# indiejoseph/speech-distill

Measured on AMD Instinct MI355X. Metric: distill-step tokens/sec (student seq_len=512), higher is better.
Workload: dtype bf16; 1 GPU; BASELINE config 2: Qwen3-0.6B-shape student + SoulX-1.7B-shape teacher (random init), V=159488, batch 4/GPU, seq_len 512, top_k 128, T=2.0 alpha=0.5, student fwd+bwd + teacher fwd + top-K + KL/CE; global_batch=4, seq_len=512, parallelism=single

## Files before the change

### speech_distill_amd/csrc/sd_attn.hip

```cpp
#include <type_traits>
#include "sd_common.cuh"
#include "../../include/sd_hip.h"
#include "sd_prof.h"
#include "sd_debug.h"
#include "sd_events.h"

namespace {

constexpr int D = 128;
constexpr int TILE = 64 * D * 2;
constexpr float NEG = -1.0e30f;
constexpr float LOG2E = 1.4426950408889634f;

SD_DEV int f_swz(int row) { return ((row & 3) << 2) | ((row >> 2) & 3); }

template <int NP = 4>
struct TileDma {
  int voff[NP];
  long row_bytes;
#if defined(__HIP_DEVICE_COMPILE__)
  __amdgpu_buffer_rsrc_t rsrc;
#endif
  SD_DEV void init(const bf16* g, long ld, int rows, int w, int lane) {
    row_bytes = ld * 2;
#if defined(__HIP_DEVICE_COMPILE__)
    rsrc = __builtin_amdgcn_make_buffer_rsrc((void*)g, 0, (int)(((long)(rows - 1) * ld + D) * 2), 0x00020000);
#endif
#pragma unroll
    for (int i = 0; i < NP; ++i) {
      const int p = (w * NP + i) * 64 + lane;
      const int row = p >> 4, s = p & 15;
      voff[i] = (int)(((long)row * ld + ((s ^ f_swz(row)) * 8)) * 2);
    }
  }
  SD_DEV void issue(int row0, char* lds, int w) const {
#if defined(__HIP_DEVICE_COMPILE__)
    const int soff = (int)(row0 * row_bytes);
#pragma unroll
    for (int i = 0; i < NP; ++i)
      __builtin_amdgcn_raw_ptr_buffer_load_lds(rsrc, (SD_LDS void*)(lds + (w * NP + i) * 1024), 16, voff[i], soff, 0, 0);
#endif
  }
};

SD_DEV bf16x8 row_frag(const char* lds, int row0, int st, int lane) {
  const int row = row0 + (lane & 31);
  const int ch = 2 * st + (lane >> 5);
  return *(const bf16x8*)(lds + row * 256 + ((ch ^ f_swz(row)) << 4));
}

SD_DEV void tr_frag4(const char* lds, int rb, int lane, bf16x8 (&out)[4]) {
  const int gi = lane >> 4, i = lane & 15, q4 = i >> 2, pp = i & 3;
  const int rA = rb + 4 * (gi >> 1) + q4, rB = rA + 8;
  const int sA = f_swz(rA), sB = f_swz(rB);
  const unsigned base = lds_addr(lds) + 8 * (pp & 1);
  const unsigned aA = base + rA * 256, aB = base + rB * 256;
  const int chl = (gi & 1) * 2 + (pp >> 1);
  sd_u64 raw[8];
#pragma unroll
  for (int db = 0; db < 4; ++db) {
    const int ch = db * 4 + chl;
    lds_tr16_pair_asm(raw[2 * db], raw[2 * db + 1], aA + ((ch ^ sA) << 4), aB + ((ch ^ sB) << 4));
  }
  lds_tr_wait8(raw);
#pragma unroll
  for (int db = 0; db < 4; ++db) out[db] = cat8_u64(raw[2 * db], raw[2 * db + 1]);
}

SD_DEV void tr_issue4(const char* lds, int rb, int lane, sd_u64 (&raw)[8]) {
  const int gi = lane >> 4, i = lane & 15, q4 = i >> 2, pp = i & 3;
  const int rA = rb + 4 * (gi >> 1) + q4, rB = rA + 8;
  const int sA = f_swz(rA), sB = f_swz(rB);
  const unsigned base = lds_addr(lds) + 8 * (pp & 1);
  const unsigned aA = base + rA * 256, aB = base + rB * 256;
  const int chl = (gi & 1) * 2 + (pp >> 1);
#pragma unroll
  for (int db = 0; db < 4; ++db) {
    const int ch = db * 4 + chl;
    lds_tr16_pair_asm(raw[2 * db], raw[2 * db + 1], aA + ((ch ^ sA) << 4), aB + ((ch ^ sB) << 4));
  }
}
SD_DEV void tr_finish4(sd_u64 (&raw)[8], bf16x8 (&out)[4]) {
  lds_tr_wait8(raw);
#pragma unroll
  for (int db = 0; db < 4; ++db) out[db] = cat8_u64(raw[2 * db], raw[2 * db + 1]);
}

SD_DEV float halves_max(float x) {
  float a = x, b = x;
  asm volatile("s_nop 1\n\tv_permlane32_swap_b32 %0, %1\n\ts_nop 0" : "+v"(a), "+v"(b));
  return fmaxf(a, b);
}

SD_DEV bf16x8 acc_frag(const f32x16& p, int s) {
  bf16x8 r;
#pragma unroll
  for (int j = 0; j < 8; ++j) r[j] = (bf16)p[8 * s + j];
  return r;
}

SD_DEV int acc_row(int reg, int h) { return (reg & 3) + 8 * (reg >> 2) + 4 * h; }

SD_DEV void store_tile_rows(char* img, const f32x16 (&acc)[4], float mul, bf16* g_row0, long ld, int rows_valid, int lane) {
  const int r = lane & 31, h = lane >> 5;
  const int swr = f_swz(r);
#pragma unroll
  for (int db = 0; db < 4; ++db)
#pragma unroll
    for (int g4 = 0; g4 < 4; ++g4) {
      bf16x4 v;
#pragma unroll
      for (int e = 0; e < 4; ++e) v[e] = (bf16)(acc[db][4 * g4 + e] * mul);
      *(bf16x4*)(img + r * 256 + (((db * 4 + g4) ^ swr) << 4) + 8 * h) = v;
    }
  asm volatile("s_waitcnt lgkmcnt(0)" ::: "memory");
  const int ch = lane & 15;
#pragma unroll
  for (int i = 0; i < 8; ++i) {
    const int row = 4 * i + (lane >> 4);
    const bf16x8 v = *(const bf16x8*)(img + row * 256 + ((ch ^ f_swz(row)) << 4));
    if (row < rows_valid) *(bf16x8*)(g_row0 + (long)row * ld + ch * 8) = v;
  }
}

struct AttnWg { int pair, member_head, hkv, b; };
SD_DEV AttnWg attn_wg(int id, int npairs, int heads_per_group, int Hkv, int B) {
  const int gs = npairs * heads_per_group, ng = Hkv * B;
  int g, mem;
  if ((ng & 7) == 0) {
    const int xcd = id & 7, slot = id >> 3;
    g = xcd + 8 * (slot / gs);
    mem = slot % gs;
  } else {
    g = id / gs;
    mem = id % gs;
  }
  AttnWg o;
  o.b = g / Hkv;
  o.hkv = g % Hkv;
  o.member_head = mem / npairs;
  o.pair = mem % npairs;
  return o;
}

#ifdef SD_STAMPS
#define SD_ATT_STAMP_PARAM , unsigned long long* stamps
#define ATT_STAMP()                                                                                   \
  do {                                                                                                \
    if (stamping && lane == 0 && sidx < 256) stamps[w8 * 256 + sidx] = __builtin_amdgcn_s_memtime();   \
    ++sidx;                                                                                           \
  } while (0)
#define ATT_STAMP_AT(COND, SLOT)                                                                            \
  do {                                                                                                      \
    if (stamping && (COND) && lane == 0) stamps[w8 * 256 + (SLOT)] = __builtin_amdgcn_s_memtime();           \
  } while (0)
#else
#define SD_ATT_STAMP_PARAM
#define ATT_STAMP() do { } while (0)
#define ATT_STAMP_AT(COND, SLOT) do { } while (0)
#endif

__global__ __launch_bounds__(512) void attn_fwd_kernel(const bf16* __restrict__ Q, const bf16* __restrict__ Kp,
                                                       const bf16* __restrict__ Vp, bf16* __restrict__ O,
                                                       float* __restrict__ LSE, const int* __restrict__ kv_len, long ldq,
                                                       long ldk, long ldv, long ldo, int T, int Hq, int Hkv,
                                                       float scale SD_ATT_STAMP_PARAM) {
  __shared__ __attribute__((aligned(16))) char smem[8 * TILE];
  const int lane = lane_id(), w8 = wave_id_uniform();
  const int n64 = (T + 63) / 64;
  const AttnWg wg = attn_wg((int)blockIdx.x, (n64 + 1) / 2, Hq / Hkv, Hkv, (int)gridDim.x / (((n64 + 1) / 2) * Hq));
#ifdef SD_STAMPS
  const bool stamping = stamps && wg.pair == 0 && wg.member_head == 0 && wg.hkv == 0 && wg.b == 0;
  int sidx = 0;
#endif
  ATT_STAMP();
  const int grp = w8 >> 2, rb = w8 & 1, half = (w8 >> 1) & 1;
  const int w = grp * 2 + rb;
  const int tA = n64 - 1 - wg.pair, tB = wg.pair;
  const bool active = grp == 0 || tB != tA;
  const int hkv = wg.hkv, b = wg.b;
  const int hq = hkv * (Hq / Hkv) + wg.member_head;
  const int q0w = (grp == 0 ? tA : tB) * 64 + 32 * rb;
  const int r = lane & 31, h = lane >> 5;
  const long tok0 = (long)b * T;
  const bf16* qb = Q + tok0 * ldq + hq * D;
  const bf16* kb = Kp + tok0 * ldk + hkv * D;
  const bf16* vb = Vp + tok0 * ldv + hkv * D;

  const int kv_hi = min(tA * 64 + 64, T);
  const int nkv = (kv_hi + 63) / 64;
  TileDma<2> kd, vd;
  kd.init(kb, ldk, T, w8, lane);
  vd.init(vb, ldv, T, w8, lane);
  kd.issue(0, smem, w8);
  vd.issue(0, smem + TILE, w8);
  const int q = q0w + r;
  const int qc = q < T ? q : T - 1;
  bf16x8 qf[8];
#pragma unroll
  for (int st = 0; st < 8; ++st) qf[st] = *(const bf16x8*)(qb + (long)qc * ldq + 16 * st + 8 * h);
  ATT_STAMP();
  const int klen = kv_len ? max(1, min(kv_len[b], T)) : T;
  const int lim = min(q, klen - 1);

  f32x16 o[4];
#pragma unroll
  for (int db = 0; db < 4; ++db)
#pragma unroll
    for (int e = 0; e < 16; ++e) o[db][e] = 0.f;
  float m = NEG, l = 0.f;
  const float c = scale * LOG2E;

  auto visible = [&](int i) { const int kv0 = i * 64 + 32 * half; return active && kv0 < kv_hi && kv0 <= q0w + 31; };
  unsigned kfo[8], vfo[2][8];
#pragma unroll
  for (int st = 0; st < 8; ++st) {
    const int row = 32 * half + (lane & 31), ch = 2 * st + (lane >> 5);
    kfo[st] = (unsigned)(row * 256 + ((ch ^ f_swz(row)) << 4));
  }
  {
    const int gi = lane >> 4, i16 = lane & 15, q4 = i16 >> 2, pp = i16 & 3;
    const int chl = (gi & 1) * 2 + (pp >> 1);
#pragma unroll
    for (int ss = 0; ss < 2; ++ss) {
      const int rA = 32 * half + 16 * ss + 4 * (gi >> 1) + q4, rB = rA + 8;
#pragma unroll
      for (int db = 0; db < 4; ++db) {
        const int ch = db * 4 + chl;
        vfo[ss][2 * db] = (unsigned)(8 * (pp & 1) + rA * 256 + ((ch ^ f_swz(rA)) << 4));
        vfo[ss][2 * db + 1] = (unsigned)(8 * (pp & 1) + rB * 256 + ((ch ^ f_swz(rB)) << 4));
      }
    }
  }
  const unsigned smem_a = lds_addr(smem);
  auto tile = [&](int i, int stage) {
    const char* ks = smem + stage * 2 * TILE;
    const unsigned vsa = smem_a + stage * 2 * TILE + TILE;
    f32x16 s1;
#pragma unroll
    for (int e = 0; e < 16; ++e) s1[e] = 0.f;
#pragma unroll
    for (int st = 0; st < 8; ++st) s1 = mfma32(*(const bf16x8*)(ks + kfo[st]), qf[st], s1);
    ATT_STAMP_AT(i == 3, 201);
    sd_u64 rv0[8], rv1[8];
#pragma unroll
    for (int db = 0; db < 4; ++db) lds_tr16_pair_asm(rv0[2 * db], rv0[2 * db + 1], vsa + vfo[0][2 * db], vsa + vfo[0][2 * db + 1]);
#pragma unroll
    for (int db = 0; db < 4; ++db) lds_tr16_pair_asm(rv1[2 * db], rv1[2 * db + 1], vsa + vfo[1][2 * db], vsa + vfo[1][2 * db + 1]);
    const int kv0 = i * 64 + 32 * half;
    const bool need_mask = __builtin_amdgcn_readfirstlane((int)((kv0 + 31 > q0w) || (kv0 + 31 >= klen))) != 0;
    if (need_mask) {
#pragma unroll
      for (int e = 0; e < 16; ++e) s1[e] = (kv0 + acc_row(e, h)) > lim ? NEG : s1[e];
    }
    float mx = fmaxf(fmaxf(s1[0], s1[1]), s1[2]);
#pragma unroll
    for (int e = 3; e < 15; e += 2) mx = fmaxf(fmaxf(mx, s1[e]), s1[e + 1]);
    mx = fmaxf(mx, s1[15]);
    ATT_STAMP_AT(i == 3, 202);
    mx = fmaxf(mx, __shfl_xor(mx, 32, 64));
    ATT_STAMP_AT(i == 3, 203);
    const float mn = fmaxf(m, mx);
    const float alpha = __builtin_amdgcn_exp2f((m - mn) * c);
    m = mn;
    const float mnc = -mn * c;
    float rs = 0.f;
#pragma unroll
    for (int e = 0; e < 16; ++e) {
      const float p = __builtin_amdgcn_exp2f(__builtin_fmaf(s1[e], c, mnc));
      s1[e] = p;
      rs += p;
    }
    l = l * alpha + rs;
    ATT_STAMP_AT(i == 3, 204);
    if (__any(alpha != 1.f)) {
#pragma unroll
      for (int db = 0; db < 4; ++db)
#pragma unroll
        for (int e = 0; e < 16; ++e) o[db][e] *= alpha;
    }
    ATT_STAMP_AT(i == 3, 205);
    bf16x8 vt[4];
    tr_finish4(rv0, vt);
    ATT_STAMP_AT(i == 3, 206);
    const bf16x8 p0 = acc_frag(s1, 0), p1 = acc_frag(s1, 1);
#pragma unroll
    for (int db = 0; db < 4; ++db) o[db] = mfma32(vt[db], p0, o[db]);
#pragma unroll
    for (int db = 0; db < 4; ++db) o[db] = mfma32(cat8_u64(rv1[2 * db], rv1[2 * db + 1]), p1, o[db]);
    ATT_STAMP_AT(i == 3, 207);
  };
  for (int i = 0; i < nkv; ++i) {
    if (i == 0) asm volatile("s_waitcnt vmcnt(0)" ::: "memory");
    else if (i + 2 < nkv) asm volatile("s_waitcnt vmcnt(8)" ::: "memory");
    else if (i + 1 < nkv) asm volatile("s_waitcnt vmcnt(4)" ::: "memory");
    else asm volatile("s_waitcnt vmcnt(0)" ::: "memory");
    ATT_STAMP();
    __builtin_amdgcn_s_barrier();
    asm volatile("" ::: "memory");
    ATT_STAMP();
    for (int t = (i == 0 ? 1 : i + 3); t <= i + 3; ++t)
      if (t < nkv) {
        char* nx = smem + (t & 3) * 2 * TILE;
        kd.issue(t * 64, nx, w8);
        vd.issue(t * 64, nx + TILE, w8);
      }
    ATT_STAMP();
    if (visible(i)) {
      ATT_STAMP_AT(i == 3, 200);
      tile(i, i & 3);
    }
    ATT_STAMP();
  }
  asm volatile("s_waitcnt vmcnt(0)" ::: "memory");
  __syncthreads();
  ATT_STAMP();
  float* xo = (float*)smem + (long)w * 66 * 64;
  if (half == 1) {
#pragma unroll
    for (int db = 0; db < 4; ++db)
#pragma unroll
      for (int e = 0; e < 16; ++e) xo[(db * 16 + e) * 64 + lane] = o[db][e];
    xo[64 * 64 + lane] = m;
    xo[65 * 64 + lane] = l;
  }
  __syncthreads();
  if (half == 1) return;
  {
    const float m1 = xo[64 * 64 + lane], l1 = xo[65 * 64 + lane];
    const float mn = fmaxf(m, m1);
    const float a0 = __builtin_amdgcn_exp2f((m - mn) * c), a1 = __builtin_amdgcn_exp2f((m1 - mn) * c);
#pragma unroll
    for (int db = 0; db < 4; ++db)
#pragma unroll
      for (int e = 0; e < 16; ++e) o[db][e] = o[db][e] * a0 + xo[(db * 16 + e) * 64 + lane] * a1;
    l = l * a0 + l1 * a1;
    m = mn;
  }
  l += __shfl_xor(l, 32, 64);
  const float inv = 1.f / l;
  ATT_STAMP();
  if (!active) return;
  store_tile_rows((char*)xo, o, inv, O + (tok0 + q0w) * ldo + hq * D, ldo, T - q0w, lane);
  if (q < T && h == 0) LSE[((long)b * Hq + hq) * T + q] = m * scale + __logf(l);
  ATT_STAMP();
}

__global__ __launch_bounds__(512) void attn_fwd_pipe_kernel(const bf16* __restrict__ Q, const bf16* __restrict__ Kp,
                                                            const bf16* __restrict__ Vp, bf16* __restrict__ O,
                                                            float* __restrict__ LSE, const int* __restrict__ kv_len,
                                                            long ldq, long ldk, long ldv, long ldo, int T, int Hq, int Hkv,
                                                            float scale SD_ATT_STAMP_PARAM) {
  __shared__ __attribute__((aligned(16))) char smem[8 * TILE];
  const int lane = lane_id(), w8 = wave_id_uniform();
  const int n64 = (T + 63) / 64;
  const AttnWg wg = attn_wg((int)blockIdx.x, (n64 + 1) / 2, Hq / Hkv, Hkv, (int)gridDim.x / (((n64 + 1) / 2) * Hq));
#ifdef SD_STAMPS
  const bool stamping = stamps && wg.pair == 0 && wg.member_head == 0 && wg.hkv == 0 && wg.b == 0;
  int sidx = 0;
#endif
  ATT_STAMP();
  const int grp = w8 >> 2, rb = w8 & 1, half = (w8 >> 1) & 1;
  const int w = grp * 2 + rb;
  const int tA = n64 - 1 - wg.pair, tB = wg.pair;
  const bool active = grp == 0 || tB != tA;
  const int hkv = wg.hkv, b = wg.b;
  const int hq = hkv * (Hq / Hkv) + wg.member_head;
  const int q0w = (grp == 0 ? tA : tB) * 64 + 32 * rb;
  const int r = lane & 31, h = lane >> 5;
  const long tok0 = (long)b * T;
  const bf16* qb = Q + tok0 * ldq + hq * D;
  const bf16* kb = Kp + tok0 * ldk + hkv * D;
  const bf16* vb = Vp + tok0 * ldv + hkv * D;
  const int kv_hi = min(tA * 64 + 64, T);
  const int nkv = (kv_hi + 63) / 64;
  TileDma<2> kd, vd;
  kd.init(kb, ldk, T, w8, lane);
  vd.init(vb, ldv, T, w8, lane);
  kd.issue(0, smem, w8);
  vd.issue(0, smem + TILE, w8);
  const int q = q0w + r;
  const int qc = q < T ? q : T - 1;
  bf16x8 qf[8];
#pragma unroll
  for (int st = 0; st < 8; ++st) qf[st] = *(const bf16x8*)(qb + (long)qc * ldq + 16 * st + 8 * h);
  const int klen = kv_len ? max(1, min(kv_len[b], T)) : T;
  const int lim = min(q, klen - 1);

  f32x16 o[4];
#pragma unroll
  for (int db = 0; db < 4; ++db)
#pragma unroll
    for (int e = 0; e < 16; ++e) o[db][e] = 0.f;
  float m = NEG, l = 0.f;
  const float c = scale * LOG2E;
  int nvis = 0;
  if (active) {
    const int last = (q0w + 31 - 32 * half) >> 6;
    nvis = (q0w + 31 - 32 * half) < 0 ? 0 : min(last + 1, (kv_hi - 32 * half + 63) >> 6);
  }
  unsigned kf0, vf0[2][2];
  {
    const int row = 32 * half + (lane & 31);
    kf0 = (unsigned)(row * 256 + (((lane >> 5) ^ f_swz(row)) << 4));
    const int gi = lane >> 4, i16 = lane & 15, q4 = i16 >> 2, pp = i16 & 3;
    const int chl = (gi & 1) * 2 + (pp >> 1);
#pragma unroll
    for (int ss = 0; ss < 2; ++ss) {
      const int rA = 32 * half + 16 * ss + 4 * (gi >> 1) + q4, rB = rA + 8;
      vf0[ss][0] = (unsigned)(8 * (pp & 1) + rA * 256 + ((chl ^ f_swz(rA)) << 4));
      vf0[ss][1] = (unsigned)(8 * (pp & 1) + rB * 256 + ((chl ^ f_swz(rB)) << 4));
    }
  }
  const unsigned smem_a = lds_addr(smem);
  auto s_tile = [&](int stage, f32x16& s) __attribute__((always_inline)) {
    const char* ks = smem + stage * 2 * TILE;
#pragma unroll
    for (int e = 0; e < 16; ++e) s[e] = 0.f;
#pragma unroll
    for (int st = 0; st < 8; ++st) s = mfma32(*(const bf16x8*)(ks + (kf0 ^ (unsigned)(st << 5))), qf[st], s);
  };
  auto mask_max = [&](int t, f32x16& s) __attribute__((always_inline)) -> float {
    const int kv0 = t * 64 + 32 * half;
    const bool need_mask = __builtin_amdgcn_readfirstlane((int)((kv0 + 31 > q0w) || (kv0 + 31 >= klen))) != 0;
    if (need_mask) {
#pragma unroll
      for (int e = 0; e < 16; ++e) s[e] = (kv0 + acc_row(e, h)) > lim ? NEG : s[e];
    }
    float mx = fmaxf(fmaxf(s[0], s[1]), s[2]);
#pragma unroll
    for (int e = 3; e < 15; e += 2) mx = fmaxf(fmaxf(mx, s[e]), s[e + 1]);
    mx = fmaxf(mx, s[15]);
    return halves_max(mx);
  };

  asm volatile("s_waitcnt vmcnt(0)" ::: "memory");
#pragma unroll
  for (int st = 0; st < 8; ++st) {
    u32x4 t4 = __builtin_bit_cast(u32x4, qf[st]);
    asm volatile("" : "+v"(t4));
    qf[st] = __builtin_bit_cast(bf16x8, t4);
  }
  __builtin_amdgcn_s_barrier();
  asm volatile("" ::: "memory");
  for (int t = 1; t <= 2; ++t)
    if (t < nkv) {
      char* nx = smem + (t & 3) * 2 * TILE;
      kd.issue(t * 64, nx, w8);
      vd.issue(t * 64, nx + TILE, w8);
    }
  f32x16 sc, sn;
  float mx = NEG;
  if (nvis > 0) {
    s_tile(0, sc);
    mx = mask_max(0, sc);
  }
  ATT_STAMP();
  for (int i = 0; i < nkv; ++i) {
    if (i + 2 < nkv) asm volatile("s_waitcnt vmcnt(4)" ::: "memory");
    else asm volatile("s_waitcnt vmcnt(0)" ::: "memory");
    ATT_STAMP();
    __builtin_amdgcn_s_barrier();
    asm volatile("" ::: "memory");
    ATT_STAMP();
    const bool comp = i < nvis;
    const unsigned ksa = smem_a + ((i + 1) & 3) * 2 * TILE + kf0;
    const unsigned vsa = smem_a + (i & 3) * 2 * TILE + TILE;
    const unsigned va[2][2] = {{vsa + vf0[0][0], vsa + vf0[0][1]}, {vsa + vf0[1][0], vsa + vf0[1][1]}};
    u32x4 kf[8];
    sd_u64 rv0[8], rv1[8];
    if (comp) {
#pragma unroll
      for (int st = 0; st < 8; ++st) asm volatile("ds_read_b128 %0, %1" : "=&v"(kf[st]) : "v"(ksa ^ (unsigned)(st << 5)));
#pragma unroll
      for (int db = 0; db < 4; ++db) lds_tr16_pair_asm(rv0[2 * db], rv0[2 * db + 1], va[0][0] ^ (unsigned)(db << 6), va[0][1] ^ (unsigned)(db << 6));
    }
    if (i + 3 < nkv) {
      char* nx = smem + ((i + 3) & 3) * 2 * TILE;
      kd.issue((i + 3) * 64, nx, w8);
      vd.issue((i + 3) * 64, nx + TILE, w8);
    }
    ATT_STAMP();
    if (!comp) {
      ATT_STAMP();
      continue;
    }
    const float mn = fmaxf(m, mx);
    const float alpha = __builtin_amdgcn_exp2f((m - mn) * c);
    m = mn;
    const float mnc = -mn * c;
    if (__any(alpha != 1.f)) {
#pragma unroll
      for (int db = 0; db < 4; ++db)
#pragma unroll
        for (int e = 0; e < 16; ++e) o[db][e] *= alpha;
    }
    asm volatile("s_waitcnt lgkmcnt(8)"
                 : "+v"(kf[0]), "+v"(kf[1]), "+v"(kf[2]), "+v"(kf[3]), "+v"(kf[4]), "+v"(kf[5]), "+v"(kf[6]), "+v"(kf[7]));
#pragma unroll
    for (int db = 0; db < 4; ++db) lds_tr16_pair_asm(rv1[2 * db], rv1[2 * db + 1], va[1][0] ^ (unsigned)(db << 6), va[1][1] ^ (unsigned)(db << 6));
#pragma unroll
    for (int e = 0; e < 16; ++e) sn[e] = 0.f;
    float rs = 0.f;
#pragma unroll
    for (int st = 0; st < 8; ++st) {
      sn = mfma32(__builtin_bit_cast(bf16x8, kf[st]), qf[st], sn);
#pragma unroll
      for (int e = 2 * st; e < 2 * st + 2; ++e) {
        const float p = __builtin_amdgcn_exp2f(__builtin_fmaf(sc[e], c, mnc));
        sc[e] = p;
        rs += p;
      }
      __builtin_amdgcn_sched_barrier(0);
    }
    l = l * alpha + rs;
    const bf16x8 p0 = acc_frag(sc, 0), p1 = acc_frag(sc, 1);
    asm volatile("s_waitcnt lgkmcnt(8)"
                 : "+v"(rv0[0]), "+v"(rv0[1]), "+v"(rv0[2]), "+v"(rv0[3]), "+v"(rv0[4]), "+v"(rv0[5]), "+v"(rv0[6]), "+v"(rv0[7]));
#pragma unroll
    for (int db = 0; db < 4; ++db) o[db] = mfma32(cat8_u64(rv0[2 * db], rv0[2 * db + 1]), p0, o[db]);
    lds_tr_wait8(rv1);
#pragma unroll
    for (int db = 0; db < 4; ++db) o[db] = mfma32(cat8_u64(rv1[2 * db], rv1[2 * db + 1]), p1, o[db]);
    mx = mask_max(i + 1, sn);
    sc = sn;
    ATT_STAMP();
  }
  asm volatile("s_waitcnt vmcnt(0)" ::: "memory");
  __syncthreads();
  ATT_STAMP();
  float* xo = (float*)smem + (long)w * 66 * 64;
  if (half == 1) {
#pragma unroll
    for (int db = 0; db < 4; ++db)
#pragma unroll
      for (int e = 0; e < 16; ++e) xo[(db * 16 + e) * 64 + lane] = o[db][e];
    xo[64 * 64 + lane] = m;
    xo[65 * 64 + lane] = l;
  }
  __syncthreads();
  if (half == 1) return;
  {
    const float m1 = xo[64 * 64 + lane], l1 = xo[65 * 64 + lane];
    const float mn = fmaxf(m, m1);
    const float a0 = __builtin_amdgcn_exp2f((m - mn) * c), a1 = __builtin_amdgcn_exp2f((m1 - mn) * c);
#pragma unroll
    for (int db = 0; db < 4; ++db)
#pragma unroll
      for (int e = 0; e < 16; ++e) o[db][e] = o[db][e] * a0 + xo[(db * 16 + e) * 64 + lane] * a1;
    l = l * a0 + l1 * a1;
    m = mn;
  }
  l += __shfl_xor(l, 32, 64);
  const float inv = 1.f / l;
  ATT_STAMP();
  if (!active) return;
  store_tile_rows((char*)xo, o, inv, O + (tok0 + q0w) * ldo + hq * D, ldo, T - q0w, lane);
  if (q < T && h == 0) LSE[((long)b * Hq + hq) * T + q] = m * scale + __logf(l);
  ATT_STAMP();
}

__global__ __launch_bounds__(256) void attn_delta_kernel(const bf16* __restrict__ dO, const bf16* __restrict__ O,
                                                         float* __restrict__ delta, long ldo, int T, int Hq, long total) {
  const int lane = lane_id();
  const long idx = ((long)blockIdx.x * 4 + (threadIdx.x >> 6)) * 4 + (lane >> 4);
  const int j = lane & 15;
  const bool ok = idx < total;
  const long id = ok ? idx : total - 1;
  const long tok = id / Hq;
  const int hh = (int)(id % Hq);
  bf16x8 a = *(const bf16x8*)(dO + tok * ldo + hh * D + j * 8);
  bf16x8 bb = *(const bf16x8*)(O + tok * ldo + hh * D + j * 8);
  float s = 0.f;
#pragma unroll
  for (int e = 0; e < 8; ++e) s += (float)a[e] * (float)bb[e];
  s += __shfl_xor(s, 1, 64); s += __shfl_xor(s, 2, 64); s += __shfl_xor(s, 4, 64); s += __shfl_xor(s, 8, 64);
  if (ok && j == 0) {
    const long bidx = tok / T;
    const int t = (int)(tok % T);
    delta[(bidx * Hq + hh) * T + t] = s;
  }
}

__global__ __launch_bounds__(512) void attn_bwd_dq_kernel(const bf16* __restrict__ Q, const bf16* __restrict__ Kp,
                                                          const bf16* __restrict__ Vp, const bf16* __restrict__ dO,
                                                          const float* __restrict__ LSE, const float* __restrict__ delta,
                                                          bf16* __restrict__ dQ, const int* __restrict__ kv_len, long ldq,
                                                          long ldk, long ldv, long ldo, long lddq, int T, int Hq, int Hkv,
                                                          float scale) {
  __shared__ __attribute__((aligned(16))) char smem[8 * TILE];
  const int lane = lane_id(), w8 = wave_id_uniform();
  const int grp = w8 >> 2, rb = w8 & 1, half = (w8 >> 1) & 1;
  const int w = grp * 2 + rb;
  const int n64 = (T + 63) / 64;
  const AttnWg wg = attn_wg((int)blockIdx.x, (n64 + 1) / 2, Hq / Hkv, Hkv, (int)gridDim.x / (((n64 + 1) / 2) * Hq));
  const int tA = n64 - 1 - wg.pair, tB = wg.pair;
  const bool active = grp == 0 || tB != tA;
  const int hkv = wg.hkv, b = wg.b;
  const int hq = hkv * (Hq / Hkv) + wg.member_head;
  const int q0w = (grp == 0 ? tA : tB) * 64 + 32 * rb;
  const int r = lane & 31, h = lane >> 5;
  const int klen = kv_len ? max(1, min(kv_len[b], T)) : T;
  const long tok0 = (long)b * T;
  const bf16* qb = Q + tok0 * ldq + hq * D;
  const bf16* kb = Kp + tok0 * ldk + hkv * D;
  const bf16* vb = Vp + tok0 * ldv + hkv * D;
  const bf16* dob = dO + tok0 * ldo + hq * D;
  const int q = q0w + r;
  const int qc = q < T ? q : T - 1;
  bf16x8 qf[8], dof[8];
#pragma unroll
  for (int st = 0; st < 8; ++st) {
    qf[st] = *(const bf16x8*)(qb + (long)qc * ldq + 16 * st + 8 * h);
    dof[st] = *(const bf16x8*)(dob + (long)qc * ldo + 16 * st + 8 * h);
  }
  const int lim = min(q, klen - 1);
  const float lse2 = LSE[((long)b * Hq + hq) * T + qc] * LOG2E;
  const float dl = delta[((long)b * Hq + hq) * T + qc];
  const float c = scale * LOG2E;
  f32x16 acc[4];
#pragma unroll
  for (int db = 0; db < 4; ++db)
#pragma unroll
    for (int e = 0; e < 16; ++e) acc[db][e] = 0.f;

  const int kv_hi = min(tA * 64 + 64, T);
  const int nkv = (kv_hi + 63) / 64;
  const int nit = (nkv + 1) >> 1;
  TileDma<> kd, vd;
  kd.init(kb, ldk, T, w, lane);
  vd.init(vb, ldv, T, w, lane);
  char* ring = smem + half * 4 * TILE;
  kd.issue(half * 64, ring, w);
  vd.issue(half * 64, ring + TILE, w);
  int cur_i = 0;
  for (int i = 0; i < nit; ++i) {
    asm volatile("s_waitcnt vmcnt(0)" ::: "memory");
    __builtin_amdgcn_s_barrier();
    asm volatile("" ::: "memory");
    if ((2 * (i + 1) + half) * 64 < kv_hi) {
      char* nx = ring + (cur_i ^ 1) * 2 * TILE;
      kd.issue((2 * (i + 1) + half) * 64, nx, w);
      vd.issue((2 * (i + 1) + half) * 64, nx + TILE, w);
    }
    const char* ks = ring + cur_i * 2 * TILE;
    const char* vs = ks + TILE;
    cur_i ^= 1;
    const int kv0 = (2 * i + half) * 64;
    if (active && kv0 < kv_hi && kv0 <= q0w + 31) {
#pragma unroll
      for (int kb2 = 0; kb2 < 2; ++kb2) {
        f32x16 s, dp;
#pragma unroll
        for (int e = 0; e < 16; ++e) { s[e] = 0.f; dp[e] = 0.f; }
#pragma unroll
        for (int st = 0; st < 8; ++st) {
          s = mfma32(row_frag(ks, kb2 * 32, st, lane), qf[st], s);
          dp = mfma32(row_frag(vs, kb2 * 32, st, lane), dof[st], dp);
        }
#pragma unroll
        for (int e = 0; e < 16; ++e) {
          const int key = kv0 + kb2 * 32 + acc_row(e, h);
          const float p = key > lim ? 0.f : __builtin_amdgcn_exp2f(s[e] * c - lse2);
          s[e] = p * (dp[e] - dl);
        }
#pragma unroll
        for (int ss = 0; ss < 2; ++ss) {
          const bf16x8 df = acc_frag(s, ss);
          bf16x8 kt4[4];
          tr_frag4(ks, kb2 * 32 + 16 * ss, lane, kt4);
#pragma unroll
          for (int db = 0; db < 4; ++db) acc[db] = mfma32(kt4[db], df, acc[db]);
        }
      }
    }
  }
  asm volatile("s_waitcnt vmcnt(0)" ::: "memory");
  __syncthreads();
  float* xo = (float*)smem + (long)w * 64 * 64;
  if (half == 1) {
#pragma unroll
    for (int db = 0; db < 4; ++db)
#pragma unroll
      for (int e = 0; e < 16; ++e) xo[(db * 16 + e) * 64 + lane] = acc[db][e];
  }
  __syncthreads();
  if (half == 1 || !active) return;
#pragma unroll
  for (int db = 0; db < 4; ++db)
#pragma unroll
    for (int e = 0; e < 16; ++e) acc[db][e] += xo[(db * 16 + e) * 64 + lane];
  store_tile_rows((char*)xo, acc, scale, dQ + (tok0 + q0w) * lddq + hq * D, lddq, T - q0w, lane);
}

__global__ __launch_bounds__(512) void attn_bwd_dkv_kernel(const bf16* __restrict__ Q, const bf16* __restrict__ Kp,
                                                           const bf16* __restrict__ Vp, const bf16* __restrict__ dO,
                                                           const float* __restrict__ LSE, const float* __restrict__ delta,
                                                           bf16* __restrict__ dK, bf16* __restrict__ dV,
                                                           const int* __restrict__ kv_len, long ldq, long ldk, long ldv,
                                                           long ldo, long lddk, long lddv, int T, int Hq, int Hkv,
                                                           float scale) {
  __shared__ __attribute__((aligned(16))) char smem[8 * TILE + 1024];
  const int lane = lane_id(), w8 = wave_id_uniform();
  const int grp = w8 >> 2, sub = w8 & 1, rh = (w8 >> 1) & 1;
  const int sw = w8 & 3;
  const int G = Hq / Hkv;
  const int n64 = (T + 63) / 64;
  const AttnWg wg = attn_wg((int)blockIdx.x, (n64 + 1) / 2, 1, Hkv, (int)gridDim.x / (((n64 + 1) / 2) * Hkv));
  const int hkv = wg.hkv, b = wg.b;
  const int kbA = wg.pair, kbB = n64 - 1 - wg.pair;
  const bool active = grp == 0 || kbB != kbA;
  const int k0w = (grp == 0 ? kbA : kbB) * 64 + 32 * sub;
  const int r = lane & 31, h = lane >> 5;
  const int klen = kv_len ? max(1, min(kv_len[b], T)) : T;
  const long tok0 = (long)b * T;
  const int key = k0w + r;
  const bool key_ok = key < klen;
  const float c = scale * LOG2E;
  char* const ksm = smem;
  char* const vsm = smem + 2 * TILE;
  char* const ring = smem + 4 * TILE;
  float* const stat = (float*)(smem + 8 * TILE);
  {
    TileDma<> kvd;
    kvd.init((grp ? Vp + tok0 * ldv : Kp + tok0 * ldk) + hkv * D, grp ? ldv : ldk, T, sw, lane);
    char* dst = grp ? vsm : ksm;
    kvd.issue(kbA * 64, dst, sw);
    kvd.issue(kbB * 64, dst + TILE, sw);
  }
  f32x16 dk[4], dv[4];
#pragma unroll
  for (int db = 0; db < 4; ++db)
#pragma unroll
    for (int e = 0; e < 16; ++e) { dk[db][e] = 0.f; dv[db][e] = 0.f; }

  const int qt0 = kbA;
  const int per_head = n64 - qt0;
  const int nit = G * per_head;
  const int st_i = threadIdx.x & 63, st_which = (threadIdx.x >> 6) & 1;
  auto load_stat = [&](int it) -> float {
    if (threadIdx.x >= 128) return 0.f;
    const int itc = it < nit ? it : nit - 1;
    const int hq = hkv * G + itc / per_head;
    int qq = (qt0 + itc % per_head) * 64 + st_i;
    qq = qq < T ? qq : T - 1;
    const long o = ((long)b * Hq + hq) * T + qq;
    return st_which ? delta[o] : LSE[o] * LOG2E;
  };
  auto stage_it = [&](int it, int buf) {
    const int g = it / per_head, qt = qt0 + it % per_head;
    const int hq = hkv * G + g;
    TileDma<> d;
    d.init((grp ? dO + tok0 * ldo : Q + tok0 * ldq) + hq * D, grp ? ldo : ldq, T, sw, lane);
    d.issue(qt * 64, ring + buf * 2 * TILE + grp * TILE, sw);
  };
  {
    const float sv0 = load_stat(0);
    stage_it(0, 0);
    if (threadIdx.x < 128) stat[st_which * 64 + st_i] = sv0;
  }
  float pend_sv = load_stat(1);
  for (int it = 0; it < nit; ++it) {
    const int buf = it & 1;
    asm volatile("s_waitcnt vmcnt(0) lgkmcnt(0)" ::: "memory");
    __builtin_amdgcn_s_barrier();
    asm volatile("" ::: "memory");
    if (threadIdx.x < 128) stat[(buf ^ 1) * 128 + st_which * 64 + st_i] = pend_sv;
    pend_sv = load_stat(it + 2);
    if (it + 1 < nit) stage_it(it + 1, buf ^ 1);
    const char* qs = ring + buf * 2 * TILE;
    const char* dos = qs + TILE;
    const int qb0 = (qt0 + it % per_head) * 64 + 32 * rh;
    if (!active || qb0 + 31 < k0w) continue;
    f32x16 s, dp;
#pragma unroll
    for (int e = 0; e < 16; ++e) { s[e] = 0.f; dp[e] = 0.f; }
#pragma unroll
    for (int st = 0; st < 8; ++st) {
      s = mfma32(row_frag(qs, 32 * rh, st, lane), row_frag(ksm, 64 * grp + 32 * sub, st, lane), s);
      dp = mfma32(row_frag(dos, 32 * rh, st, lane), row_frag(vsm, 64 * grp + 32 * sub, st, lane), dp);
    }
#pragma unroll
    for (int g4 = 0; g4 < 4; ++g4) {
      const f32x4 l2 = *(const f32x4*)&stat[buf * 128 + 32 * rh + 8 * g4 + 4 * h];
      const f32x4 dl = *(const f32x4*)&stat[buf * 128 + 64 + 32 * rh + 8 * g4 + 4 * h];
#pragma unroll
      for (int e = 0; e < 4; ++e) {
        const int qq = qb0 + 8 * g4 + 4 * h + e;
        const bool vis = key_ok && key <= qq && qq < T;
        const float p = vis ? __builtin_amdgcn_exp2f(s[4 * g4 + e] * c - l2[e]) : 0.f;
        s[4 * g4 + e] = p;
        dp[4 * g4 + e] = p * (dp[4 * g4 + e] - dl[e]);
      }
    }
#pragma unroll
    for (int ss = 0; ss < 2; ++ss) {
      bf16x8 t4[4];
      const bf16x8 pf = acc_frag(s, ss);
      tr_frag4(dos, 32 * rh + 16 * ss, lane, t4);
#pragma unroll
      for (int db = 0; db < 4; ++db) dv[db] = mfma32(t4[db], pf, dv[db]);
      const bf16x8 df = acc_frag(dp, ss);
      tr_frag4(qs, 32 * rh + 16 * ss, lane, t4);
#pragma unroll
      for (int db = 0; db < 4; ++db) dk[db] = mfma32(t4[db], df, dk[db]);
    }
  }
  asm volatile("s_waitcnt vmcnt(0) lgkmcnt(0)" ::: "memory");
  __syncthreads();
  float* xo = (float*)smem + (long)(grp * 2 + sub) * 64 * 64;
#pragma unroll
  for (int round = 0; round < 2; ++round) {
    f32x16* acc = round ? dv : dk;
    if (rh == 1) {
#pragma unroll
      for (int db = 0; db < 4; ++db)
#pragma unroll
        for (int e = 0; e < 16; ++e) xo[(db * 16 + e) * 64 + lane] = acc[db][e];
    }
    __syncthreads();
    if (rh == 0) {
#pragma unroll
      for (int db = 0; db < 4; ++db)
#pragma unroll
        for (int e = 0; e < 16; ++e) acc[db][e] += xo[(db * 16 + e) * 64 + lane];
    }
    __syncthreads();
  }
  if (rh == 0 && active) {
    store_tile_rows((char*)xo, dk, scale, dK + (tok0 + k0w) * lddk + hkv * D, lddk, T - k0w, lane);
    store_tile_rows((char*)xo + 8192, dv, 1.f, dV + (tok0 + k0w) * lddv + hkv * D, lddv, T - k0w, lane);
  }
}

int check_common(int B, int T, int Hq, int Hkv, long ldq, long ldk, long ldv, long ldo) {
  if (B <= 0 || T <= 0 || Hq <= 0 || Hkv <= 0 || (Hq % Hkv)) return SD_ERR_SHAPE;
  if ((ldq | ldk | ldv | ldo) & 7) return SD_ERR_ALIGN;
  return 0;
}

}

#ifdef SD_STAMPS
static unsigned long long* g_attn_stamps = nullptr;
extern "C" void sd_debug_attn_stamp_buffer(void* p) { g_attn_stamps = (unsigned long long*)p; }
#define SD_ATT_STAMP_ARG , g_attn_stamps
#else
#define SD_ATT_STAMP_ARG
#endif


extern "C" int sd_attn_fwd(const void* q, const void* k, const void* v, void* o, float* lse, const int32_t* kv_len,
                           int64_t ldq, int64_t ldk, int64_t ldv, int64_t ldo, int B, int T, int Hq, int Hkv,
                           int head_dim, float scale, void* stream) {
  if (head_dim != D) return SD_ERR_UNSUPPORTED;
  if (int e = check_common(B, T, Hq, Hkv, ldq, ldk, ldv, ldo)) return e;
  if (((uintptr_t)q | (uintptr_t)k | (uintptr_t)v | (uintptr_t)o) & 15) return SD_ERR_ALIGN;
  SdProfScope prof(SD_K_ATTN_FWD, 2.0 * B * Hq * (double)T * T * D, (hipStream_t)stream);
  const dim3 grid((((T + 63) / 64 + 1) / 2) * Hq * B);
  const bool pipe = (g_sd_debug.attn_variant & 2) || (!(g_sd_debug.attn_variant & 1) && T >= 1024);
  if (pipe) {
    hipLaunchKernelGGL(attn_fwd_pipe_kernel, grid, dim3(512), 0, (hipStream_t)stream, (const bf16*)q, (const bf16*)k,
                       (const bf16*)v, (bf16*)o, lse, kv_len, ldq, ldk, ldv, ldo, T, Hq, Hkv, scale SD_ATT_STAMP_ARG);
    SD_CHECK_LAUNCH();
    return 0;
  }
  hipLaunchKernelGGL(attn_fwd_kernel, grid, dim3(512), 0, (hipStream_t)stream, (const bf16*)q,
                     (const bf16*)k, (const bf16*)v, (bf16*)o, lse, kv_len, ldq, ldk, ldv, ldo, T, Hq, Hkv, scale SD_ATT_STAMP_ARG);
  SD_CHECK_LAUNCH();
  return 0;
}

extern "C" int sd_attn_bwd2(const void* q, const void* k, const void* v, const void* o, const void* d_o, const float* lse,
                            float* delta, void* dq, void* dk, void* dv, const int32_t* kv_len, int64_t ldq, int64_t ldk,
                            int64_t ldv, int64_t ldo, int64_t lddq, int64_t lddk, int64_t lddv, int B, int T, int Hq,
                            int Hkv, int head_dim, float scale, void* side_stream, void* stream) {
  if (head_dim != D) return SD_ERR_UNSUPPORTED;
  if (int e = check_common(B, T, Hq, Hkv, ldq, ldk, ldv, ldo)) return e;
  if ((lddq | lddk | lddv) & 7) return SD_ERR_ALIGN;
  hipStream_t st = (hipStream_t)stream, s2 = (hipStream_t)side_stream;
  SdEventLease lease;
  if (s2 && !(lease.set = sd_lease_events())) return SD_ERR_WORKSPACE;
  hipEvent_t* g_attn_ev = lease.set ? lease.set->ev : nullptr;
  const long total = (long)B * T * Hq;
  if (o) {
    hipLaunchKernelGGL(attn_delta_kernel, dim3((unsigned)((total + 15) / 16)), dim3(256), 0, st, (const bf16*)d_o,
                       (const bf16*)o, delta, ldo, T, Hq, total);
    SD_CHECK_LAUNCH();
  }
  hipStream_t sq = s2 ? s2 : st;
  if (s2) {
    if (hipEventRecord(g_attn_ev[0], st) != hipSuccess || hipStreamWaitEvent(s2, g_attn_ev[0], 0) != hipSuccess)
      return SD_ERR_WORKSPACE;
  }
  {
    SdProfScope prof2(SD_K_ATTN_BWD_DQ, 3.0 * B * Hq * (double)T * T * D, sq);
    hipLaunchKernelGGL(attn_bwd_dq_kernel, dim3((((T + 63) / 64 + 1) / 2) * Hq * B), dim3(512), 0, sq, (const bf16*)q, (const bf16*)k,
                       (const bf16*)v, (const bf16*)d_o, lse, (const float*)delta, (bf16*)dq, kv_len, ldq, ldk, ldv, ldo,
                       lddq, T, Hq, Hkv, scale);
  }
  SD_CHECK_LAUNCH();
  {
    SdProfScope prof(SD_K_ATTN_BWD_DKV, 4.0 * B * Hq * (double)T * T * D, st);
    hipLaunchKernelGGL(attn_bwd_dkv_kernel, dim3((((T + 63) / 64 + 1) / 2) * Hkv * B), dim3(512), 0, st, (const bf16*)q,
                       (const bf16*)k, (const bf16*)v, (const bf16*)d_o, lse, (const float*)delta, (bf16*)dk, (bf16*)dv,
                       kv_len, ldq, ldk, ldv, ldo, lddk, lddv, T, Hq, Hkv, scale);
  }
  SD_CHECK_LAUNCH();
  if (s2) {
    if (hipEventRecord(g_attn_ev[1], s2) != hipSuccess || hipStreamWaitEvent(st, g_attn_ev[1], 0) != hipSuccess)
      return SD_ERR_WORKSPACE;
  }
  return 0;
}

extern "C" int sd_attn_bwd(const void* q, const void* k, const void* v, const void* o, const void* d_o, const float* lse,
                           float* delta, void* dq, void* dk, void* dv, const int32_t* kv_len, int64_t ldq, int64_t ldk,
                           int64_t ldv, int64_t ldo, int64_t lddq, int64_t lddk, int64_t lddv, int B, int T, int Hq,
                           int Hkv, int head_dim, float scale, void* stream) {
  return sd_attn_bwd2(q, k, v, o, d_o, lse, delta, dq, dk, dv, kv_len, ldq, ldk, ldv, ldo, lddq, lddk, lddv, B, T, Hq,
                      Hkv, head_dim, scale, nullptr, stream);
}
```

Measured before the change: 102,000 tokens/s.

## Restructure attention dKV backward: one key block per workgroup, split query tiles across halves

The dK/dV backward kernel now assigns one 64-key block per workgroup instead of pairing two key blocks. The two wave halves process alternating query tiles (Q and dO staged together) and their partial sums are reduced through shared memory at the end. LSE and delta are read straight from global memory with vectorized loads, replacing the shared-memory stat staging. The change also interleaves the exp2 computation with the dP MFMAs, skips masking on interior tiles, and launches dKV before dQ. Grid size doubles, while the final reduction and shared memory use both grow, and load balance now depends on causal tile counts per block.

```diff
diff --git a/speech_distill_amd/csrc/sd_attn.hip b/speech_distill_amd/csrc/sd_attn.hip
--- a/speech_distill_amd/csrc/sd_attn.hip
+++ b/speech_distill_amd/csrc/sd_attn.hip
@@ -693,6 +693,7 @@
   store_tile_rows((char*)xo, acc, scale, dQ + (tok0 + q0w) * lddq + hq * D, lddq, T - q0w, lane);
 }
 
+template <bool STAT_VEC>
 __global__ __launch_bounds__(512) void attn_bwd_dkv_kernel(const bf16* __restrict__ Q, const bf16* __restrict__ Kp,
                                                            const bf16* __restrict__ Vp, const bf16* __restrict__ dO,
                                                            const float* __restrict__ LSE, const float* __restrict__ delta,
@@ -700,17 +701,15 @@
                                                            const int* __restrict__ kv_len, long ldq, long ldk, long ldv,
                                                            long ldo, long lddk, long lddv, int T, int Hq, int Hkv,
                                                            float scale) {
-  __shared__ __attribute__((aligned(16))) char smem[8 * TILE + 1024];
+  __shared__ __attribute__((aligned(16))) char smem[10 * TILE];
   const int lane = lane_id(), w8 = wave_id_uniform();
-  const int grp = w8 >> 2, sub = w8 & 1, rh = (w8 >> 1) & 1;
+  const int part = w8 >> 2, sub = w8 & 1, rh = (w8 >> 1) & 1;
   const int sw = w8 & 3;
   const int G = Hq / Hkv;
   const int n64 = (T + 63) / 64;
-  const AttnWg wg = attn_wg((int)blockIdx.x, (n64 + 1) / 2, 1, Hkv, (int)gridDim.x / (((n64 + 1) / 2) * Hkv));
-  const int hkv = wg.hkv, b = wg.b;
-  const int kbA = wg.pair, kbB = n64 - 1 - wg.pair;
-  const bool active = grp == 0 || kbB != kbA;
-  const int k0w = (grp == 0 ? kbA : kbB) * 64 + 32 * sub;
+  const AttnWg wg = attn_wg((int)blockIdx.x, n64, 1, Hkv, (int)gridDim.x / (n64 * Hkv));
+  const int hkv = wg.hkv, b = wg.b, kb = wg.pair;
+  const int k0w = kb * 64 + 32 * sub;
   const int r = lane & 31, h = lane >> 5;
   const int klen = kv_len ? max(1, min(kv_len[b], T)) : T;
   const long tok0 = (long)b * T;
@@ -718,81 +717,99 @@
   const bool key_ok = key < klen;
   const float c = scale * LOG2E;
   char* const ksm = smem;
-  char* const vsm = smem + 2 * TILE;
-  char* const ring = smem + 4 * TILE;
-  float* const stat = (float*)(smem + 8 * TILE);
+  char* const vsm = smem + TILE;
+  char* const ring = smem + 2 * TILE;
   {
     TileDma<> kvd;
-    kvd.init((grp ? Vp + tok0 * ldv : Kp + tok0 * ldk) + hkv * D, grp ? ldv : ldk, T, sw, lane);
-    char* dst = grp ? vsm : ksm;
-    kvd.issue(kbA * 64, dst, sw);
-    kvd.issue(kbB * 64, dst + TILE, sw);
-  }
+    kvd.init((part ? Vp + tok0 * ldv : Kp + tok0 * ldk) + hkv * D, part ? ldv : ldk, T, sw, lane);
+    kvd.issue(kb * 64, part ? vsm : ksm, sw);
+  }
+  const int per_head = n64 - kb;
+  const int nvis = G * per_head;
+  const int nit = (nvis + 1) >> 1;
+  auto stage = [&](int v, int buf) {
+    const int hq = hkv * G + v / per_head, q0 = (kb + v % per_head) * 64;
+    char* dst = ring + (buf * 2 + part) * 2 * TILE;
+    TileDma<> d;
+    d.init(Q + tok0 * ldq + hq * D, ldq, T, sw, lane);
+    d.issue(q0, dst, sw);
+    d.init(dO + tok0 * ldo + hq * D, ldo, T, sw, lane);
+    d.issue(q0, dst + TILE, sw);
+  };
+  stage(min(part, nvis - 1), 0);
   f32x16 dk[4], dv[4];
 #pragma unroll
   for (int db = 0; db < 4; ++db)
 #pragma unroll
     for (int e = 0; e < 16; ++e) { dk[db][e] = 0.f; dv[db][e] = 0.f; }
 
-  const int qt0 = kbA;
-  const int per_head = n64 - qt0;
-  const int nit = G * per_head;
-  const int st_i = threadIdx.x & 63, st_which = (threadIdx.x >> 6) & 1;
-  auto load_stat = [&](int it) -> float {
-    if (threadIdx.x >= 128) return 0.f;
-    const int itc = it < nit ? it : nit - 1;
-    const int hq = hkv * G + itc / per_head;
-    int qq = (qt0 + itc % per_head) * 64 + st_i;
-    qq = qq < T ? qq : T - 1;
-    const long o = ((long)b * Hq + hq) * T + qq;
-    return st_which ? delta[o] : LSE[o] * LOG2E;
+  const unsigned qfo = (unsigned)((32 * rh + r) * 256 + ((h ^ f_swz(32 * rh + r)) << 4));
+  const unsigned kfo = (unsigned)((32 * sub + r) * 256 + ((h ^ f_swz(32 * sub + r)) << 4));
+  auto stat_wait = [](f32x4 (&l4)[4], f32x4 (&d4)[4]) __attribute__((always_inline)) {
+    asm volatile("s_waitcnt vmcnt(8)"
+                 : "+v"(l4[0]), "+v"(l4[1]), "+v"(l4[2]), "+v"(l4[3]), "+v"(d4[0]), "+v"(d4[1]), "+v"(d4[2]), "+v"(d4[3]));
   };
-  auto stage_it = [&](int it, int buf) {
-    const int g = it / per_head, qt = qt0 + it % per_head;
-    const int hq = hkv * G + g;
-    TileDma<> d;
-    d.init((grp ? dO + tok0 * ldo : Q + tok0 * ldq) + hq * D, grp ? ldo : ldq, T, sw, lane);
-    d.issue(qt * 64, ring + buf * 2 * TILE + grp * TILE, sw);
-  };
-  {
-    const float sv0 = load_stat(0);
-    stage_it(0, 0);
-    if (threadIdx.x < 128) stat[st_which * 64 + st_i] = sv0;
-  }
-  float pend_sv = load_stat(1);
-  for (int it = 0; it < nit; ++it) {
-    const int buf = it & 1;
+  for (int j = 0; j < nit; ++j) {
+    const int buf = j & 1;
+    const int v = 2 * j + part;
+    const int vc = v < nvis ? v : nvis - 1;
+    const int qb0 = (kb + vc % per_head) * 64 + 32 * rh;
     asm volatile("s_waitcnt vmcnt(0) lgkmcnt(0)" ::: "memory");
+    const long so = ((long)b * Hq + hkv * G + vc / per_head) * T;
+    f32x4 l4[4], d4[4];
+    if constexpr (STAT_VEC) {
+#pragma unroll
+      for (int g4 = 0; g4 < 4; ++g4) {
+        const int r4 = min(qb0 + 8 * g4 + 4 * h, T - 4);
+        asm volatile("global_load_dwordx4 %0, %1, off" : "=v"(l4[g4]) : "v"(LSE + so + r4));
+        asm volatile("global_load_dwordx4 %0, %1, off" : "=v"(d4[g4]) : "v"(delta + so + r4));
+      }
+    }
     __builtin_amdgcn_s_barrier();
     asm volatile("" ::: "memory");
-    if (threadIdx.x < 128) stat[(buf ^ 1) * 128 + st_which * 64 + st_i] = pend_sv;
-    pend_sv = load_stat(it + 2);
-    if (it + 1 < nit) stage_it(it + 1, buf ^ 1);
-    const char* qs = ring + buf * 2 * TILE;
+    stage(min(v + 2, nvis - 1), buf ^ 1);
+    const bool dead = v >= nvis || qb0 + 31 < k0w;
+    const char* qs = ring + (buf * 2 + part) * 2 * TILE;
     const char* dos = qs + TILE;
-    const int qb0 = (qt0 + it % per_head) * 64 + 32 * rh;
-    if (!active || qb0 + 31 < k0w) continue;
+    unsigned qo = qfo, ko = kfo;
+    asm volatile("" : "+v"(qo), "+v"(ko));
     f32x16 s, dp;
 #pragma unroll
     for (int e = 0; e < 16; ++e) { s[e] = 0.f; dp[e] = 0.f; }
 #pragma unroll
+    for (int st = 0; st < 8; ++st)
+      s = mfma32(*(const bf16x8*)(qs + (qo ^ (unsigned)(st << 5))), *(const bf16x8*)(ksm + (ko ^ (unsigned)(st << 5))), s);
+    const bool need_mask =
+        __builtin_amdgcn_readfirstlane((int)(dead || (qb0 < k0w + 31) || (qb0 + 31 >= T) || (k0w + 31 >= klen))) != 0;
+    if (need_mask) {
+#pragma unroll
+      for (int e = 0; e < 16; ++e) {
+        const int qq = qb0 + acc_row(e, h);
+        s[e] = (!dead && key_ok && key <= qq && qq < T) ? s[e] : NEG;
+      }
+    }
+    float nl2[16], dl[16];
+    if constexpr (STAT_VEC) {
+      stat_wait(l4, d4);
+#pragma unroll
+      for (int e = 0; e < 16; ++e) { nl2[e] = l4[e >> 2][e & 3] * -LOG2E; dl[e] = d4[e >> 2][e & 3]; }
+    } else {
+#pragma unroll
+      for (int e = 0; e < 16; ++e) {
+        const int qq = min(qb0 + acc_row(e, h), T - 1);
+        nl2[e] = LSE[so + qq] * -LOG2E;
+        dl[e] = delta[so + qq];
+      }
+    }
+#pragma unroll
     for (int st = 0; st < 8; ++st) {
-      s = mfma32(row_frag(qs, 32 * rh, st, lane), row_frag(ksm, 64 * grp + 32 * sub, st, lane), s);
-      dp = mfma32(row_frag(dos, 32 * rh, st, lane), row_frag(vsm, 64 * grp + 32 * sub, st, lane), dp);
-    }
-#pragma unroll
-    for (int g4 = 0; g4 < 4; ++g4) {
-      const f32x4 l2 = *(const f32x4*)&stat[buf * 128 + 32 * rh + 8 * g4 + 4 * h];
-      const f32x4 dl = *(const f32x4*)&stat[buf * 128 + 64 + 32 * rh + 8 * g4 + 4 * h];
-#pragma unroll
-      for (int e = 0; e < 4; ++e) {
-        const int qq = qb0 + 8 * g4 + 4 * h + e;
-        const bool vis = key_ok && key <= qq && qq < T;
-        const float p = vis ? __builtin_amdgcn_exp2f(s[4 * g4 + e] * c - l2[e]) : 0.f;
-        s[4 * g4 + e] = p;
-        dp[4 * g4 + e] = p * (dp[4 * g4 + e] - dl[e]);
-      }
-    }
+      dp = mfma32(*(const bf16x8*)(dos + (qo ^ (unsigned)(st << 5))), *(const bf16x8*)(vsm + (ko ^ (unsigned)(st << 5))), dp);
+#pragma unroll
+      for (int e = 2 * st; e < 2 * st + 2; ++e) s[e] = __builtin_amdgcn_exp2f(__builtin_fmaf(s[e], c, nl2[e]));
+      __builtin_amdgcn_sched_barrier(0);
+    }
+#pragma unroll
+    for (int e = 0; e < 16; ++e) dp[e] = s[e] * (dp[e] - dl[e]);
 #pragma unroll
     for (int ss = 0; ss < 2; ++ss) {
       bf16x8 t4[4];
@@ -808,28 +825,57 @@
   }
   asm volatile("s_waitcnt vmcnt(0) lgkmcnt(0)" ::: "memory");
   __syncthreads();
-  float* xo = (float*)smem + (long)(grp * 2 + sub) * 64 * 64;
-#pragma unroll
-  for (int round = 0; round < 2; ++round) {
-    f32x16* acc = round ? dv : dk;
-    if (rh == 1) {
+  {
+    float* const x1 = (float*)smem + (long)(rh * 2 + sub) * 2 * 4096;
+    if (part == 1) {
 #pragma unroll
       for (int db = 0; db < 4; ++db)
 #pragma unroll
-        for (int e = 0; e < 16; ++e) xo[(db * 16 + e) * 64 + lane] = acc[db][e];
+        for (int e = 0; e < 16; ++e) {
+          x1[(db * 16 + e) * 64 + lane] = dk[db][e];
+          x1[4096 + (db * 16 + e) * 64 + lane] = dv[db][e];
+        }
     }
     __syncthreads();
-    if (rh == 0) {
+    if (part == 0) {
 #pragma unroll
       for (int db = 0; db < 4; ++db)
 #pragma unroll
-        for (int e = 0; e < 16; ++e) acc[db][e] += xo[(db * 16 + e) * 64 + lane];
+        for (int e = 0; e < 16; ++e) {
+          dk[db][e] += x1[(db * 16 + e) * 64 + lane];
+          dv[db][e] += x1[4096 + (db * 16 + e) * 64 + lane];
+        }
     }
     __syncthreads();
   }
-  if (rh == 0 && active) {
-    store_tile_rows((char*)xo, dk, scale, dK + (tok0 + k0w) * lddk + hkv * D, lddk, T - k0w, lane);
-    store_tile_rows((char*)xo + 8192, dv, 1.f, dV + (tok0 + k0w) * lddv + hkv * D, lddv, T - k0w, lane);
+  float* const x2 = (float*)smem + (long)sub * 2 * 4096;
+  if (part == 1) {
+  } else if (rh == 1) {
+#pragma unroll
+    for (int db = 0; db < 4; ++db)
+#pragma unroll
+      for (int e = 0; e < 16; ++e) x2[(db * 16 + e) * 64 + lane] = dk[db][e];
+  } else {
+#pragma unroll
+    for (int db = 0; db < 4; ++db)
+#pragma unroll
+      for (int e = 0; e < 16; ++e) x2[4096 + (db * 16 + e) * 64 + lane] = dv[db][e];
+  }
+  __syncthreads();
+  if (part == 1) return;
+  char* const img = smem + 4 * TILE + w8 * 8192;
+  if (rh == 0) {
+#pragma unroll
+    for (int db = 0; db < 4; ++db)
+#pragma unroll
+      for (int e = 0; e < 16; ++e) dk[db][e] += x2[(db * 16 + e) * 64 + lane];
+    store_tile_rows(img, dk, scale, dK + (tok0 + k0w) * lddk + hkv * D, lddk, T - k0w, lane);
+  } else {
+#pragma unroll
+    for (int db = 0; db < 4; ++db)
+#pragma unroll
+      for (int e = 0; e < 16; ++e) dv[db][e] += x2[4096 + (db * 16 + e) * 64 + lane];
+    store_tile_rows(img, dv, 1.f, dV + (tok0 + k0w) * lddv + hkv * D, lddv, T - k0w, lane);
   }
 }
 
@@ -894,17 +940,18 @@
       return SD_ERR_WORKSPACE;
   }
   {
+    SdProfScope prof(SD_K_ATTN_BWD_DKV, 4.0 * B * Hq * (double)T * T * D, st);
+    const bool stat_vec = (T & 3) == 0 && !(((uintptr_t)lse | (uintptr_t)delta) & 15);
+    hipLaunchKernelGGL(stat_vec ? attn_bwd_dkv_kernel<true> : attn_bwd_dkv_kernel<false>, dim3(((T + 63) / 64) * Hkv * B),
+                       dim3(512), 0, st, (const bf16*)q, (const bf16*)k, (const bf16*)v, (const bf16*)d_o, lse,
+                       (const float*)delta, (bf16*)dk, (bf16*)dv, kv_len, ldq, ldk, ldv, ldo, lddk, lddv, T, Hq, Hkv, scale);
+  }
+  SD_CHECK_LAUNCH();
+  {
     SdProfScope prof2(SD_K_ATTN_BWD_DQ, 3.0 * B * Hq * (double)T * T * D, sq);
     hipLaunchKernelGGL(attn_bwd_dq_kernel, dim3((((T + 63) / 64 + 1) / 2) * Hq * B), dim3(512), 0, sq, (const bf16*)q, (const bf16*)k,
                        (const bf16*)v, (const bf16*)d_o, lse, (const float*)delta, (bf16*)dq, kv_len, ldq, ldk, ldv, ldo,
                        lddq, T, Hq, Hkv, scale);
-  }
-  SD_CHECK_LAUNCH();
-  {
-    SdProfScope prof(SD_K_ATTN_BWD_DKV, 4.0 * B * Hq * (double)T * T * D, st);
-    hipLaunchKernelGGL(attn_bwd_dkv_kernel, dim3((((T + 63) / 64 + 1) / 2) * Hkv * B), dim3(512), 0, st, (const bf16*)q,
-                       (const bf16*)k, (const bf16*)v, (const bf16*)d_o, lse, (const float*)delta, (bf16*)dk, (bf16*)dv,
-                       kv_len, ldq, ldk, ldv, ldo, lddk, lddv, T, Hq, Hkv, scale);
   }
   SD_CHECK_LAUNCH();
   if (s2) {
```

After: 100,900 tokens/s (median of 2 runs). 1.1% lower.
